# facebookresearch/AVID-CMA

Hardware: AMD Instinct MI355X
Metric: clips/sec (video+audio fwd+bwd+NCE+Adam) (higher is better)
Workload: dtype f32 (bf16x3 MFMA)

## Files before the change

### avid-cma_amd/csrc/conv.hip

```cpp
#include <math.h>
#include <stdlib.h>

#include <atomic>
#include <type_traits>

#include "common.h"

namespace avid {

typedef unsigned int uintx4 __attribute__((ext_vector_type(4)));

struct ConvArgs {
  const float* __restrict__ src;
  const float* __restrict__ wk;
  int w_row, w_nrec;
  const float* __restrict__ addend;
  const float* __restrict__ bias;
  float* __restrict__ dst;
  float* __restrict__ part;
  int B, Ts, Hs, Ws, Cs;
  int Td, Hd, Wd, Cd;
  int kt, kh, kw;
  int st, sh, sw;
  int pt, ph, pw;
// ... 704 lines not shown
#pragma unroll
        for (int j = 0; j < TN; ++j) {
          const pk_bf16x8 bh = bq[st & 1][j][0], bm = bq[st & 1][j][1], bl = bq[st & 1][j][2];
#pragma unroll
          for (int i = 0; i < TM; ++i) {
            acc[i][j] = __builtin_amdgcn_mfma_f32_32x32x16_bf16(ah[i], bl, acc[i][j], 0, 0, 0);
            acc[i][j] = __builtin_amdgcn_mfma_f32_32x32x16_bf16(al[i], bh, acc[i][j], 0, 0, 0);
            acc[i][j] = __builtin_amdgcn_mfma_f32_32x32x16_bf16(am[i], bm, acc[i][j], 0, 0, 0);
            acc[i][j] = __builtin_amdgcn_mfma_f32_32x32x16_bf16(ah[i], bm, acc[i][j], 0, 0, 0);
            acc[i][j] = __builtin_amdgcn_mfma_f32_32x32x16_bf16(am[i], bh, acc[i][j], 0, 0, 0);
            acc[i][j] = __builtin_amdgcn_mfma_f32_32x32x16_bf16(ah[i], bh, acc[i][j], 0, 0, 0);
          }
        }
      }
      return;
    }
    if (PK_SPLIT && TM * TN >= 4) {
      const float* As = Ab - h * 4 + h * 8;
      const float* Bs = Bb - h * 4 + h * 8;
#pragma unroll
      for (int st = 0; st < BK / 16; ++st) {
        if (decltype(ST)::value && st == 0) store_stage(nxt);
        if (decltype(LD)::value && st == 1) issue_loads();
        pk_bf16x8 ah[TM], am[TM], al[TM];
#pragma unroll
        for (int i = 0; i < TM; ++i) {
          const floatx4 v0 = *reinterpret_cast<const floatx4*>(As + i * 32 * LDK + st * 16);
          const floatx4 v1 = *reinterpret_cast<const floatx4*>(As + i * 32 * LDK + st * 16 + 4);
          pk_split8(v0, v1, ah[i], am[i], al[i]);
        }
#pragma unroll
        for (int j = 0; j < TN; ++j) {
          const floatx4 v0 = *reinterpret_cast<const floatx4*>(Bs + j * 32 * LDK + st * 16);
          const floatx4 v1 = *reinterpret_cast<const floatx4*>(Bs + j * 32 * LDK + st * 16 + 4);
          pk_bf16x8 bh, bm, bl;
          pk_split8(v0, v1, bh, bm, bl);
#pragma unroll
          for (int i = 0; i < TM; ++i) {
            acc[i][j] = __builtin_amdgcn_mfma_f32_32x32x16_bf16(ah[i], bl, acc[i][j], 0, 0, 0);
            acc[i][j] = __builtin_amdgcn_mfma_f32_32x32x16_bf16(al[i], bh, acc[i][j], 0, 0, 0);
            acc[i][j] = __builtin_amdgcn_mfma_f32_32x32x16_bf16(am[i], bm, acc[i][j], 0, 0, 0);
            acc[i][j] = __builtin_amdgcn_mfma_f32_32x32x16_bf16(ah[i], bm, acc[i][j], 0, 0, 0);
            acc[i][j] = __builtin_amdgcn_mfma_f32_32x32x16_bf16(am[i], bh, acc[i][j], 0, 0, 0);
            acc[i][j] = __builtin_amdgcn_mfma_f32_32x32x16_bf16(ah[i], bh, acc[i][j], 0, 0, 0);
          }
        }
      }
      return;
    }
    floatx4 af[2][TM], bf[2][TN];
#pragma unroll
    for (int i = 0; i < TM; ++i) af[0][i] = *reinterpret_cast<const floatx4*>(Ab + i * 32 * LDK);
#pragma unroll
    for (int j = 0; j < TN; ++j) bf[0][j] = *reinterpret_cast<const floatx4*>(Bb + j * 32 * LDK);
#pragma unroll
    for (int g = 0; g < BK / 8; ++g) {
      if (g + 1 < BK / 8) {
#pragma unroll
        for (int i = 0; i < TM; ++i)
          af[(g + 1) & 1][i] = *reinterpret_cast<const floatx4*>(Ab + i * 32 * LDK + (g + 1) * 8);
#pragma unroll
        for (int j = 0; j < TN; ++j)
          bf[(g + 1) & 1][j] = *reinterpret_cast<const floatx4*>(Bb + j * 32 * LDK + (g + 1) * 8);
      }
      __builtin_amdgcn_sched_barrier(0);
      if (decltype(ST)::value && g == 0) store_stage(nxt);
      if (decltype(LD)::value && g == 1) issue_loads();
#pragma unroll
      for (int s = 0; s < 4; ++s)
#pragma unroll
        for (int i = 0; i < TM; ++i)
#pragma unroll
          for (int j = 0; j < TN; ++j)
            acc[i][j] = __builtin_amdgcn_mfma_f32_32x32x2f32(af[g & 1][i][s], bf[g & 1][j][s], acc[i][j], 0, 0, 0);
      if (decltype(ST)::value && g == 0) {
#pragma unroll
        for (int q = 0; q < PA + PB; ++q) {
          __builtin_amdgcn_sched_group_barrier(0x008, 1, 0);
          __builtin_amdgcn_sched_group_barrier(0x200, 1, 0);
        }
      }
      if (decltype(LD)::value && g == 1) {
#pragma unroll
        for (int q = 0; q < PA + PB; ++q) {
          __builtin_amdgcn_sched_group_barrier(0x008, 1, 0);
          __builtin_amdgcn_sched_group_barrier(0x020, 1, 0);
        }
      }
      __builtin_amdgcn_sched_barrier(0);
    }
  };

  const int row_bytes = p.Cd * 4;
  for (int j = 0; j < nseg; ++j) {
    int tile, k0, k1, split;
    seg_info(j, tile, k0, k1, split);
    const int nkj = k1 - k0;
#pragma unroll
    for (int i = 0; i < TM; ++i)
#pragma unroll
      for (int jj = 0; jj < TN; ++jj)
#pragma unroll
        for (int r = 0; r < 16; ++r) acc[i][jj][r] = 0.f;

    int nst = left - 2 < nkj ? left - 2 : nkj;
    if (nst < 0) nst = 0;
    PK_STAMP(2 + 3 * j);
    for (int ks = 0; ks < nst; ++ks, u ^= 1) {
      ktile(std::true_type{}, std::true_type{});
      advance();
      __syncthreads();
    }
    left -= nst;
    if (nst < nkj) {
      if (left == 2) {
        ktile(std::true_type{}, std::false_type{});
        __syncthreads();
        u ^= 1;
        --left;
        ++nst;
      }
      if (nst < nkj) {
        ktile(std::false_type{}, std::false_type{});
        __syncthreads();
        u ^= 1;
        --left;
      }
    }

    PK_STAMP(3 + 3 * j);
    if (STRIDED) {
      int* drow = reinterpret_cast<int*>(smem + 2 * STAGE);
      int* arow = drow + BM;
      const bool sparse_add = p.add_s[0] * p.add_s[1] * p.add_s[2] > 1;
      const int c = cls_of(tile);
      const int lt = tile - kp->cls_begin[c];
      const int mt = lt / ntn, nt = lt - mt * ntn;
      const int n0 = nt * BN;
      const int cT = kp->cls_n[c][0], cH = kp->cls_n[c][1], cW = kp->cls_n[c][2];
      __syncthreads();
      if (tid < BM) {
        const unsigned m = mt * BM + tid;
        const bool ok = m < (unsigned)(p.B * cT * cH * cW);
        const unsigned mm = ok ? m : 0u;
        const unsigned q1 = magic_div(mm, kp->cls_mg[c][2], kp->cls_shf[c][2]);
        const int wd = mm - q1 * cW;
        const unsigned q2 = magic_div(q1, kp->cls_mg[c][1], kp->cls_shf[c][1]);
        const int hd = q1 - q2 * cH;
        const int b = magic_div(q2, kp->cls_mg[c][0], kp->cls_shf[c][0]);
        const int td = q2 - b * cT;
        const int dst = ((b * p.Td + kp->cls_p0[c][0] + td * p.st) * p.Hd + kp->cls_p0[c][1] + hd * p.sh) * p.Wd +
                        kp->cls_p0[c][2] + wd * p.sw;
        drow[tid] = ok ? dst * row_bytes : (int)OOB;
        if (sparse_add) {
          const int t = kp->cls_p0[c][0] + td * p.st, hh = kp->cls_p0[c][1] + hd * p.sh, w = kp->cls_p0[c][2] + wd * p.sw;
          const bool on = ok && (t & (p.add_s[0] - 1)) == 0 && (hh & (p.add_s[1] - 1)) == 0 && (w & (p.add_s[2] - 1)) == 0;
          const int ar = ((b * p.add_n[0] + (t >> (p.add_s[0] - 1))) * p.add_n[1] + (hh >> (p.add_s[1] - 1))) * p.add_n[2] +
                         (w >> (p.add_s[2] - 1));
          arow[tid] = on ? ar * row_bytes : (int)OOB;
        } else {
          arow[tid] = ok ? dst * row_bytes : (int)OOB;
        }
      }
      __syncthreads();
      const bool direct = split < 0;
      const __amdgpu_buffer_rsrc_t rsD = __builtin_amdgcn_make_buffer_rsrc(
          (void*)(direct ? p.dst : p.part + (long long)split * p.M * p.Cd), 0, (int)((long long)p.M * row_bytes), 0x00020000);
      const long long add_rows = sparse_add ? (long long)p.B * p.add_n[0] * p.add_n[1] * p.add_n[2] : (long long)p.M;
      const __amdgpu_buffer_rsrc_t rsE = __builtin_amdgcn_make_buffer_rsrc(
          (void*)(p.addend ? p.addend : p.dst), 0, (int)(add_rows * row_bytes), 0x00020000);
      const __amdgpu_buffer_rsrc_t rsXb = __builtin_amdgcn_make_buffer_rsrc(
          (void*)(p.bnb_x ? p.bnb_x : p.dst), 0, (int)((long long)p.M * row_bytes), 0x00020000);
      auto emit = [&](auto HAS_ADD, auto BNB) {
#pragma unroll
        for (int i = 0; i < TM; ++i) {
#pragma unroll
          for (int jj = 0; jj < TN; ++jj) {
            const int col = n0 + (wn * TN + jj) * 32 + l31;
            const int col4 = col * 4;
            unsigned voff[16];
            float ad[16], xb[16], bsc = 0.f, bsh = 0.f, bmu = 0.f, bis = 0.f;
#pragma unroll
            for (int r = 0; r < 16; ++r) {
              const int trow = (wm * TM + i) * 32 + (r & 3) + 8 * (r >> 2) + 4 * h;
              voff[r] = (unsigned)drow[trow] + col4;
              if (HAS_ADD)
                ad[r] = __builtin_bit_cast(float, __builtin_amdgcn_raw_buffer_load_b32(rsE, (unsigned)arow[trow] + col4, 0, 0));
              if (BNB) xb[r] = __builtin_bit_cast(float, __builtin_amdgcn_raw_buffer_load_b32(rsXb, voff[r], 0, 0));
            }
            if (BNB) { bsc = p.bnb_scale[col]; bsh = p.bnb_shift[col]; bmu = p.bnb_mean[col]; bis = p.bnb_invstd[col]; }
#pragma unroll
            for (int r = 0; r < 16; ++r) {
              float v = acc[i][jj][r];
              if (HAS_ADD) v += ad[r];
              if (BNB) {
                const float dm = (!p.bnb_relu || fmaf(xb[r], bsc, bsh) > 0.f) ? v : 0.f;
                cs[jj][r & 1] += dm;
                cq[jj][r & 1] = fmaf(dm, (xb[r] - bmu) * bis, cq[jj][r & 1]);
              }
              __builtin_amdgcn_raw_buffer_store_b32(__builtin_bit_cast(unsigned, v), rsD, voff[r], 0, 0);
            }
          }
        }
      };
      constexpr std::true_type Y{};
      constexpr std::false_type N{};
      if (!direct) emit(N, N);
      else if (EPI == 9) emit(Y, Y);
      else if (EPI == 8) emit(N, Y);
      else if (EPI == 1) emit(Y, N);
      else if (EPI == 0) emit(N, N);
      else if (p.bnb_x) { if (p.addend) emit(Y, Y); else emit(N, Y); }
      else if (p.addend) emit(Y, N);
      else emit(N, N);
      continue;
    }
    const int mt = tile / ntn, nt = tile - mt * ntn;
    const int m0 = mt * BM, n0 = nt * BN;
    int rows = p.M - m0;
    rows = rows > BM ? BM : rows;
    const bool direct = split < 0;
    const long long d_base = (long long)m0 * p.Cd;
    const long long s_base = ((long long)split * (p.M - p.part_row_begin) + (m0 - p.part_row_begin)) * p.Cd;
    const __amdgpu_buffer_rsrc_t rsD = __builtin_amdgcn_make_buffer_rsrc(
        (void*)(direct ? p.dst + d_base : p.part + s_base), 0, rows * row_bytes, 0x00020000);
    const __amdgpu_buffer_rsrc_t rsE = __builtin_amdgcn_make_buffer_rsrc(
        (void*)(p.addend ? p.addend + d_base : p.dst + d_base), 0, rows * row_bytes, 0x00020000);
    const __amdgpu_buffer_rsrc_t rsXb = __builtin_amdgcn_make_buffer_rsrc(
        (void*)(p.bnb_x ? p.bnb_x + d_base : p.dst + d_base), 0, rows * row_bytes, 0x00020000);
    auto emit = [&](auto DIRECT, auto HAS_ADD, auto RELU, auto OP, auto BNB, auto BIAS) {
#pragma unroll
      for (int i = 0; i < TM; ++i) {
#pragma unroll
        for (int jj = 0; jj < TN; ++jj) {
          const int col = n0 + (wn * TN + jj) * 32 + l31;
          const unsigned voff = (unsigned)(((wm * TM + i) * 32 + 4 * h) * p.Cd + col) * 4;
          float ad[16];
          if (HAS_ADD) {
#pragma unroll
            for (int r = 0; r < 16; ++r)
              ad[r] = __builtin_bit_cast(float, __builtin_amdgcn_raw_buffer_load_b32(
                                                    rsE, voff, ((r & 3) + 8 * (r >> 2)) * row_bytes, 0));
          }
          const float bv = (DIRECT && decltype(BIAS)::value != 0 && (decltype(BIAS)::value == 1 || p.bias)) ? p.bias[col] : 0.f;
          float xb[16], bsc = 0.f, bsh = 0.f, bmu = 0.f, bis = 0.f;
          if (BNB) {
#pragma unroll
            for (int r = 0; r < 16; ++r)
              xb[r] = __builtin_bit_cast(float, __builtin_amdgcn_raw_buffer_load_b32(
                                                    rsXb, voff, ((r & 3) + 8 * (r >> 2)) * row_bytes, 0));
            bsc = p.bnb_scale[col]; bsh = p.bnb_shift[col]; bmu = p.bnb_mean[col]; bis = p.bnb_invstd[col];
          }
#pragma unroll
          for (int r = 0; r < 16; ++r) {
            const int soff = ((r & 3) + 8 * (r >> 2)) * row_bytes;
            float v = acc[i][jj][r];
            if (DIRECT) {
              if (decltype(BIAS)::value != 0) v += bv;
              if (HAS_ADD) v = decltype(OP)::value == 0 ? v + ad[r] : (decltype(OP)::value == 1 ? fminf(v, ad[r]) : fmaxf(v, ad[r]));
              if (RELU) v = fmaxf(v, 0.f);
              if (MODE == 0) { cs[jj][r & 1] += v; cq[jj][r & 1] = fmaf(v, v, cq[jj][r & 1]); }
              if (BNB) {
                const float dm = (!p.bnb_relu || fmaf(xb[r], bsc, bsh) > 0.f) ? v : 0.f;
                cs[jj][r & 1] += dm;
                cq[jj][r & 1] = fmaf(dm, (xb[r] - bmu) * bis, cq[jj][r & 1]);
              }
            }
            __builtin_amdgcn_raw_buffer_store_b32(__builtin_bit_cast(unsigned, v), rsD, voff, soff, 0);
          }
        }
      }
    };
    constexpr std::true_type Y{};
    constexpr std::false_type N{};
    constexpr std::integral_constant<int, 0> ADD{};
    constexpr std::integral_constant<int, 0> B0{};
    constexpr std::integral_constant<int, 1> B1{};
    constexpr std::integral_constant<int, 2> BQ{};
    if (!direct) emit(N, N, N, ADD, N, B0);
    else if (EPI == 0) emit(Y, N, N, ADD, N, B0);
    else if (EPI == 1) emit(Y, Y, N, ADD, N, B0);
    else if (MODE == 0 && EPI == 2) emit(Y, N, N, ADD, N, B1);
    else if (MODE == 0 && EPI == 3) emit(Y, N, Y, ADD, N, B1);
    else if (MODE == 0 && EPI == 4) emit(Y, Y, N, std::integral_constant<int, 1>{}, N, B0);
    else if (MODE == 0 && EPI == 5) emit(Y, Y, N, std::integral_constant<int, 2>{}, N, B0);
    else if (MODE == 1 && EPI == 8) emit(Y, N, N, ADD, Y, B0);
    else if (MODE == 1 && EPI == 9) emit(Y, Y, N, ADD, Y, B0);
    else if (MODE == 1 && p.bnb_x) {
      if (p.addend) emit(Y, Y, N, ADD, Y, BQ); else emit(Y, N, N, ADD, Y, BQ);
    } else if (p.addend) {
      if (MODE == 0 && p.epi_op == 1) emit(Y, Y, N, std::integral_constant<int, 1>{}, N, BQ);
      else if (MODE == 0 && p.epi_op == 2) emit(Y, Y, N, std::integral_constant<int, 2>{}, N, BQ);
      else if (p.relu) emit(Y, Y, Y, ADD, N, BQ);
      else emit(Y, Y, N, ADD, N, BQ);
    } else {
      if (p.relu) emit(Y, N, Y, ADD, N, BQ); else emit(Y, N, N, ADD, N, BQ);
    }
    PK_STAMP(4 + 3 * j);
  }
  write_stats();
  PK_STAMP(31);
}

constexpr int WG_LD_C = 64 + 4;
constexpr int TC_P = 32;
constexpr int TC_T = 8;
constexpr int TC_ROWS = TC_P * TC_T;
constexpr int TC_B_BYTES = 6 * PK_BCH;
constexpr int TC_STAGE = TC_ROWS * LDK;
constexpr size_t TC_LDS = TC_B_BYTES + (2 * TC_STAGE + TC_P * LDK + 128) * sizeof(float);

template <int MODE, int EPI, bool AFF = false>
__global__ __launch_bounds__(512) __attribute__((amdgpu_waves_per_eu(2, 2))) void tconv64_kernel(const ConvArgs p) {
  constexpr bool OAFF = (EPI & 2) != 0;
  static_assert(!AFF || MODE == 0, "the input affine map belongs to the forward");
  static_assert(!OAFF || (MODE == 0 && (EPI & 8) == 0), "the output affine map belongs to the forward");
  extern __shared__ __attribute__((aligned(16))) float smem[];
  char* Bs = reinterpret_cast<char*>(smem);
  float* As = smem + TC_B_BYTES / 4;
  const int tid = threadIdx.x, lane = tid & 63;
  const int wave = __builtin_amdgcn_readfirstlane(tid >> 6);
  const int h = lane >> 5, l31 = lane & 31;
  const int lcol = (tid & 7) * 4;
  const int G = gridDim.x;
  const int slot = __builtin_amdgcn_readfirstlane((int)xcd_remap(blockIdx.x, G));
  PK_STAMP(0);
  const int HW = p.Hs * p.Ws;
  const int NP = p.B * HW;
  const int ntiles = (NP + TC_P - 1) / TC_P;
  const int nmine = slot < ntiles ? (ntiles - slot + G - 1) / G : 0;
  const int nitems = 2 * nmine;
  const int frame_bytes = HW * 256;

  float cs[2][2], cq[2][2];
#pragma unroll
  for (int j = 0; j < 2; ++j) cs[j][0] = cs[j][1] = cq[j][0] = cq[j][1] = 0.f;
  auto write_stats = [&]() {
    if (OAFF || !p.stats) return;
    float* red = As;
    __syncthreads();
#pragma unroll
    for (int j = 0; j < 2; ++j) {
      const float a0 = cs[j][0] + cs[j][1], b0 = cq[j][0] + cq[j][1];
      const float a = a0 + __shfl_xor(a0, 32, 64), b = b0 + __shfl_xor(b0, 32, 64);
      if (h == 0) {
        red[wave * 64 + j * 32 + l31] = a;
        red[512 + wave * 64 + j * 32 + l31] = b;
      }
    }
    __syncthreads();
    if (tid < 128) {
      const int c = tid & 63, which = tid >> 6;
      float a = 0.f;
#pragma unroll
      for (int w = 0; w < 8; ++w) a += red[which * 512 + w * 64 + c];
      p.stats[(long long)slot * 128 + which * 64 + c] = a;
      for (int r = slot + G; r < p.stats_rows; r += G) p.stats[(long long)r * 128 + which * 64 + c] = 0.f;
    }
  };
  if (nitems == 0) {
    write_stats();
    return;
  }

  const __amdgpu_buffer_rsrc_t rsA = __builtin_amdgcn_make_buffer_rsrc(
      (void*)p.src, 0, (int)((long long)p.M * 256), 0x00020000);
  const bool lead = wave < 4;
  const int trow = (tid & 255) >> 3;
  unsigned ld_voff = OOB;
  auto ld_tile = [&](int li) {
    const int tile = slot + (li >> 1) * G;
    const unsigned pg = (unsigned)(tile * TC_P + trow);
    const unsigned b = magic_div(pg, p.mgW, p.shW);
    const unsigned hw = pg - b * HW;
    ld_voff = pg < (unsigned)NP ? (unsigned)((b * TC_T * HW + hw) * 256 + lcol * 4) : OOB;
  };
  floatx4 va[8];
  auto issue_loads = [&](int li) {
    const int c128 = (li & 1) * 128;
#pragma unroll
    for (int i = 0; i < 8; ++i)
      va[i] = __builtin_bit_cast(floatx4, __builtin_amdgcn_raw_buffer_load_b128(
                                              rsA, ld_voff, __builtin_amdgcn_readfirstlane(c128 + i * frame_bytes), 0));
  };
  const float* aff = As + 2 * TC_STAGE + TC_P * LDK;
  auto store_stage = [&](float* st, int blk, bool first = false) {
    floatx4 asc = {0.f, 0.f, 0.f, 0.f}, ash = asc;
    if (AFF) {
      if (first) {
        asc = *reinterpret_cast<const floatx4*>(p.in_scale + blk * 32 + lcol);
        ash = *reinterpret_cast<const floatx4*>(p.in_shift + blk * 32 + lcol);
      } else {
        asc = *reinterpret_cast<const floatx4*>(aff + blk * 32 + lcol);
        ash = *reinterpret_cast<const floatx4*>(aff + 64 + blk * 32 + lcol);
      }
    }
#pragma unroll
    for (int i = 0; i < 8; ++i) {
      floatx4 v = va[i];
      if (AFF) {
        const bool ok = ld_voff != OOB;
#pragma unroll
        for (int j = 0; j < 4; ++j) {
          float o = fmaf(v[j], asc[j], ash[j]);
          if (p.in_relu) o = fmaxf(o, 0.f);
          v[j] = ok ? o : 0.f;
        }
      }
      *reinterpret_cast<floatx4*>(&st[(trow + 32 * i) * LDK + lcol]) = v;
    }
  };

  if (lead) {
    const __amdgpu_buffer_rsrc_t rsB = __builtin_amdgcn_make_buffer_rsrc(const_cast<void*>(p.wsp), 0, TC_B_BYTES, 0x00020000);
    pk_uintx4 wv[18];
#pragma unroll
    for (int i = 0; i < 18; ++i)
      wv[i] = __builtin_bit_cast(pk_uintx4, __builtin_amdgcn_raw_buffer_load_b128(rsB, (tid + 256 * i) * 16, 0, 0));
    for (int i = tid; i < TC_P * LDK; i += 256) As[2 * TC_STAGE + i] = 0.f;
    if (AFF && tid < 128) As[2 * TC_STAGE + TC_P * LDK + tid] = tid < 64 ? p.in_scale[tid] : p.in_shift[tid - 64];
#pragma unroll
    for (int i = 0; i < 18; ++i) *reinterpret_cast<pk_uintx4*>(Bs + (tid + 256 * i) * 16) = wv[i];
  } else {
    ld_tile(0);
    issue_loads(0);
    store_stage(As, 0, true);
    if (nitems > 1) issue_loads(1);
  }
  __syncthreads();

  floatx16 acc[2];
  const int row_bytes = 256;
  const __amdgpu_buffer_rsrc_t rsD = __builtin_amdgcn_make_buffer_rsrc((void*)p.dst, 0, (int)((long long)p.M * row_bytes), 0x00020000);
  const __amdgpu_buffer_rsrc_t rsE = __builtin_amdgcn_make_buffer_rsrc(
      (void*)(p.addend ? p.addend : p.dst), 0, (int)((long long)p.M * row_bytes), 0x00020000);
  const __amdgpu_buffer_rsrc_t rsXb = __builtin_amdgcn_make_buffer_rsrc(
      (void*)(p.bnb_x ? p.bnb_x : p.dst), 0, (int)((long long)p.M * row_bytes), 0x00020000);
  constexpr bool HAS_ADD = (EPI & 1) != 0, BNB = (EPI & 8) != 0;
  float bsc[2] = {0.f, 0.f}, bsh[2] = {0.f, 0.f}, bmu[2] = {0.f, 0.f}, bis[2] = {0.f, 0.f};
  if (BNB) {
#pragma unroll
    for (int j = 0; j < 2; ++j) {
      const int col = j * 32 + l31;
      bsc[j] = p.bnb_scale[col]; bsh[j] = p.bnb_shift[col]; bmu[j] = p.bnb_mean[col]; bis[j] = p.bnb_invstd[col];
    }
  }
  float osc[2] = {0.f, 0.f}, osh[2] = {0.f, 0.f};
  if (OAFF) {
#pragma unroll
    for (int j = 0; j < 2; ++j) {
      osc[j] = p.bnb_scale[j * 32 + l31];
      osh[j] = p.bnb_shift[j * 32 + l31];
    }
  }

  const float* Alane = As + l31 * LDK + h * 8;
  auto products = [&](int stage_off, auto CB) {
    constexpr int cb = decltype(CB)::value;
    int aoff[3];
#pragma unroll
    for (int d = 0; d < 3; ++d) {
      const int f = MODE == 0 ? wave + d - 1 : wave + 1 - d;
      aoff[d] = __builtin_amdgcn_readfirstlane((f < 0 || f >= TC_T) ? 2 * TC_STAGE : stage_off + f * TC_P * LDK);
    }
    const float* Af[3] = {Alane + aoff[0], Alane + aoff[1], Alane + aoff[2]};
    const char* Bc = Bs + cb * PK_BCH + lane * 16;
    floatx4 ar[3][2];
    pk_bf16x8 bf[3][6], sp[2][3];
    auto request = [&](int s_, int buf) {
      const int d = s_ >> 1, st = s_ & 1;
      ar[buf][0] = *reinterpret_cast<const floatx4*>(Af[d] + st * 16);
      ar[buf][1] = *reinterpret_cast<const floatx4*>(Af[d] + st * 16 + 4);
#pragma unroll
      for (int j = 0; j < 2; ++j)
#pragma unroll
        for (int t = 0; t < 3; ++t)
          bf[buf][j * 3 + t] = *reinterpret_cast<const pk_bf16x8*>(Bc + d * 2 * PK_BCH + ((j * 2 + st) * 3 + t) * 1024);
    };
    request(0, 0);
    request(1, 1);
    pk_split8<false>(ar[0][0], ar[0][1], sp[0][0], sp[0][1], sp[0][2]);
    __builtin_amdgcn_sched_barrier(0);
#pragma unroll
    for (int s_ = 0; s_ < 6; ++s_) {
      const int b = s_ % 3, q2 = s_ & 1;
      if (s_ + 2 < 6) request(s_ + 2, (s_ + 2) % 3);
      if (s_ + 1 < 6) pk_split8<false>(ar[(s_ + 1) % 3][0], ar[(s_ + 1) % 3][1], sp[q2 ^ 1][0], sp[q2 ^ 1][1], sp[q2 ^ 1][2]);
      const pk_bf16x8 ah = sp[q2][0], am = sp[q2][1], al = sp[q2][2];
      acc[0] = __builtin_amdgcn_mfma_f32_32x32x16_bf16(ah, bf[b][2], acc[0], 0, 0, 0);
      acc[1] = __builtin_amdgcn_mfma_f32_32x32x16_bf16(ah, bf[b][5], acc[1], 0, 0, 0);
      acc[0] = __builtin_amdgcn_mfma_f32_32x32x16_bf16(al, bf[b][0], acc[0], 0, 0, 0);
      acc[1] = __builtin_amdgcn_mfma_f32_32x32x16_bf16(al, bf[b][3], acc[1], 0, 0, 0);
      acc[0] = __builtin_amdgcn_mfma_f32_32x32x16_bf16(am, bf[b][1], acc[0], 0, 0, 0);
      acc[1] = __builtin_amdgcn_mfma_f32_32x32x16_bf16(am, bf[b][4], acc[1], 0, 0, 0);
      acc[0] = __builtin_amdgcn_mfma_f32_32x32x16_bf16(ah, bf[b][1], acc[0], 0, 0, 0);
      acc[1] = __builtin_amdgcn_mfma_f32_32x32x16_bf16(ah, bf[b][4], acc[1], 0, 0, 0);
      acc[0] = __builtin_amdgcn_mfma_f32_32x32x16_bf16(am, bf[b][0], acc[0], 0, 0, 0);
      acc[1] = __builtin_amdgcn_mfma_f32_32x32x16_bf16(am, bf[b][3], acc[1], 0, 0, 0);
      acc[0] = __builtin_amdgcn_mfma_f32_32x32x16_bf16(ah, bf[b][0], acc[0], 0, 0, 0);
      acc[1] = __builtin_amdgcn_mfma_f32_32x32x16_bf16(ah, bf[b][3], acc[1], 0, 0, 0);
      if (s_ + 2 < 6) __builtin_amdgcn_sched_group_barrier(0x100, 8, 0);
#pragma unroll
      for (int q = 0; q < 12; ++q) {
        __builtin_amdgcn_sched_group_barrier(0x008, 1, 0);
        if (s_ + 1 < 6) __builtin_amdgcn_sched_group_barrier(0x002, 3, 0);
      }
      __builtin_amdgcn_sched_barrier(0);
    }
  };

  auto emit = [&](int tile, const floatx16 (&res)[2], auto SPLIT) {
    const unsigned p0 = (unsigned)(tile * TC_P);
    const unsigned b0 = magic_div(p0, p.mgW, p.shW);
    const unsigned pb = (b0 + 1) * HW;
    const unsigned base = (p0 + (7 * b0 + wave) * HW) * 256u + l31 * 4 + h * 4 * 256;
    const unsigned step_b = 7u * HW * 256u;
    unsigned voff[16];
#pragma unroll
    for (int r = 0; r < 16; ++r) {
      voff[r] = base;
      if (decltype(SPLIT)::value) {
        const unsigned pg = p0 + (r & 3) + 8 * (r >> 2) + 4 * h;
        voff[r] = pg < (unsigned)NP ? base + (pg >= pb ? step_b : 0u) : OOB;
      }
    }
#pragma unroll
    for (int j = 0; j < 2; ++j) {
      float ad[16], xb[16];
      if (HAS_ADD) {
#pragma unroll
        for (int r = 0; r < 16; ++r)
          ad[r] = __builtin_bit_cast(float, __builtin_amdgcn_raw_buffer_load_b32(rsE, voff[r], ((r & 3) + 8 * (r >> 2)) * 256 + j * 128, 0));
      }
      if (BNB) {
#pragma unroll
        for (int r = 0; r < 16; ++r)
          xb[r] = __builtin_bit_cast(float, __builtin_amdgcn_raw_buffer_load_b32(rsXb, voff[r], ((r & 3) + 8 * (r >> 2)) * 256 + j * 128, 0));
      }
#pragma unroll
      for (int r = 0; r < 16; ++r) {
        float v = res[j][r];
        if (HAS_ADD) v += ad[r];
        if (OAFF) {
          v = fmaf(v, osc[j], osh[j]);
          if (p.bnb_relu) v = fmaxf(v, 0.f);
        } else if (MODE == 0) { cs[j][r & 1] += v; cq[j][r & 1] = fmaf(v, v, cq[j][r & 1]); }
        if (BNB) {
          const float dm = (!p.bnb_relu || fmaf(xb[r], bsc[j], bsh[j]) > 0.f) ? v : 0.f;
          cs[j][r & 1] += dm;
          cq[j][r & 1] = fmaf(dm, (xb[r] - bmu[j]) * bis[j], cq[j][r & 1]);
        }
        __builtin_amdgcn_raw_buffer_store_b32(__builtin_bit_cast(unsigned, v), rsD, voff[r], ((r & 3) + 8 * (r >> 2)) * 256 + j * 128, 0);
      }
    }
  };
  auto epilogue = [&](int tile, const floatx16 (&res)[2]) {
    const unsigned p0 = (unsigned)(tile * TC_P);
    const unsigned pb = (magic_div(p0, p.mgW, p.shW) + 1) * HW;
    if (p0 + TC_P <= pb && p0 + TC_P <= (unsigned)NP) emit(tile, res, std::false_type{});
    else emit(tile, res, std::true_type{});
  };
  auto stage_next = [&](int it, int cb) {
    if (it + 1 < nitems) store_stage(As + (cb ^ 1) * TC_STAGE, cb ^ 1);
    if (it + 2 < nitems) {
      if (cb == 0) ld_tile(it + 2);
      issue_loads(it + 2);
    }
  };
  floatx16 out[2];
  PK_STAMP(1);
  for (int t = 0; t < nmine; ++t) {
    PK_STAMP(2 + 7 * t);
    if (!lead) {
      stage_next(2 * t, 0);
      if (t > 0) epilogue(slot + (t - 1) * G, out);
    }
#pragma unroll
    for (int j = 0; j < 2; ++j)
#pragma unroll
      for (int r = 0; r < 16; ++r) acc[j][r] = 0.f;
    PK_STAMP(3 + 7 * t);
#ifdef AVID_PK_TRACE
    if (t == 3 && lane == 0) g_pk_trace[(512 + blockIdx.x) * 64 + wave] = wall_clock64();
#endif
    products(0, std::integral_constant<int, 0>{});
#ifdef AVID_PK_TRACE
    if (t == 3 && lane == 0) g_pk_trace[(512 + blockIdx.x) * 64 + 8 + wave] = wall_clock64();
#endif
    PK_STAMP(4 + 7 * t);
    __syncthreads();
    PK_STAMP(5 + 7 * t);
    if (!lead) stage_next(2 * t + 1, 1);
    products(TC_STAGE, std::integral_constant<int, 1>{});
    PK_STAMP(6 + 7 * t);
    if (lead) {
      epilogue(slot + t * G, acc);
    } else {
      out[0] = acc[0];
      out[1] = acc[1];
    }
    PK_STAMP(7 + 7 * t);
    __syncthreads();
    PK_STAMP(8 + 7 * t);
  }
  if (!lead) epilogue(slot + (nmine - 1) * G, out);
  PK_STAMP(31);
  write_stats();
}

constexpr int TWG_P = 16;
constexpr int TWG_PLANE = TC_T * TWG_P * WG_LD_C;
constexpr size_t TWG_LDS = sizeof(float) * 2 * 2 * TWG_PLANE;

struct TwgradArgs {
  const float* x; const float* dy; float* part;
  int B, HW;
  unsigned mg; int sh;
  const float* in_scale; const float* in_shift;
  int in_relu;
};

template <bool AFF>
__global__ __launch_bounds__(512) __attribute__((amdgpu_waves_per_eu(2, 2))) void twgrad64_kernel(const TwgradArgs p) {
  extern __shared__ __attribute__((aligned(16))) float smem[];
  const int tid = threadIdx.x, lane = tid & 63;
  const int wave = __builtin_amdgcn_readfirstlane(tid >> 6);
  const int h = lane >> 5, l31 = lane & 31;
  const int jn = wave & 1, jc = (wave >> 1) & 1, kh = wave >> 2;
  const int G = gridDim.x;
  const int slot = __builtin_amdgcn_readfirstlane((int)xcd_remap(blockIdx.x, G));
  const int HW = p.HW, NP = p.B * HW;
  const int ntiles = (NP + TWG_P - 1) / TWG_P;
  const int nmine = slot < ntiles ? (ntiles - slot + G - 1) / G : 0;
  const int frame_bytes = HW * 256;
  const long long total = (long long)NP * TC_T * 256;
  const __amdgpu_buffer_rsrc_t rsX = __builtin_amdgcn_make_buffer_rsrc((void*)p.x, 0, (int)total, 0x00020000);
  const __amdgpu_buffer_rsrc_t rsY = __builtin_amdgcn_make_buffer_rsrc((void*)p.dy, 0, (int)total, 0x00020000);
  const int trow = tid >> 4, lcol = (tid & 15) * 4;
  unsigned ld_voff = OOB;
  auto ld_tile = [&](int k) {
    const unsigned pg = (unsigned)((slot + k * G) * TWG_P + (trow & 15));
    const unsigned b = magic_div(pg, p.mg, p.sh);
    const unsigned hw = pg - b * HW;
    ld_voff = pg < (unsigned)NP ? (unsigned)(((b * TC_T + (trow >> 4)) * HW + hw) * 256 + lcol * 4) : OOB;
  };
  floatx4 vx[4], vy[4];
  auto issue_loads = [&]() {
#pragma unroll
    for (int i = 0; i < 4; ++i) {
      const int so = __builtin_amdgcn_readfirstlane(2 * i * frame_bytes);
      vy[i] = __builtin_bit_cast(floatx4, __builtin_amdgcn_raw_buffer_load_b128(rsY, ld_voff, so, 0));
      vx[i] = __builtin_bit_cast(floatx4, __builtin_amdgcn_raw_buffer_load_b128(rsX, ld_voff, so, 0));
    }
  };
  floatx4 asc = {0.f, 0.f, 0.f, 0.f}, ash = asc;
  if (AFF) {
    asc = *reinterpret_cast<const floatx4*>(p.in_scale + lcol);
    ash = *reinterpret_cast<const floatx4*>(p.in_shift + lcol);
  }
  auto store_stage = [&](float* st) {
#pragma unroll
    for (int i = 0; i < 4; ++i) {
      floatx4 v = vx[i];
      if (AFF) {
        const bool ok = ld_voff != OOB;
#pragma unroll
        for (int j = 0; j < 4; ++j) {
          float o = fmaf(v[j], asc[j], ash[j]);
          if (p.in_relu) o = fmaxf(o, 0.f);
          v[j] = ok ? o : 0.f;
        }
      }
      *reinterpret_cast<floatx4*>(&st[(trow + 32 * i) * WG_LD_C + lcol]) = vy[i];
      *reinterpret_cast<floatx4*>(&st[TWG_PLANE + (trow + 32 * i) * WG_LD_C + lcol]) = v;
    }
  };
  floatx16 acc[3];
#pragma unroll
  for (int d = 0; d < 3; ++d)
#pragma unroll
    for (int r = 0; r < 16; ++r) acc[d][r] = 0.f;
  if (nmine > 0) {
    ld_tile(0);
    issue_loads();
    store_stage(smem);
    if (nmine > 1) { ld_tile(1); issue_loads(); }
  }
  __syncthreads();
  auto frag = [&](const float* plane, int f, int col, pk_bf16x8& fh, pk_bf16x8& fm, pk_bf16x8& fl) {
    const float* q = plane + (f * TWG_P + h * 8) * WG_LD_C + col;
    float v[8];
#pragma unroll
    for (int i = 0; i < 8; ++i) v[i] = q[i * WG_LD_C];
    pk_split8<true>(floatx4{v[0], v[1], v[2], v[3]}, floatx4{v[4], v[5], v[6], v[7]}, fh, fm, fl);
  };
  const int ncol = jn * 32 + l31, ccol = jc * 32 + l31;
  const int t0 = kh * 4;
  for (int k = 0; k < nmine; ++k) {
    const float* cur = smem + (k & 1) * 2 * TWG_PLANE;
    float* nxt = smem + ((k + 1) & 1) * 2 * TWG_PLANE;
    if (k + 1 < nmine) store_stage(nxt);
    if (k + 2 < nmine) { ld_tile(k + 2); issue_loads(); }
    const float* Dp = cur;
    const float* Xp = cur + TWG_PLANE;
    pk_bf16x8 xw[3][3];
    if (t0 > 0) frag(Xp, t0 - 1, ccol, xw[0][0], xw[0][1], xw[0][2]);
    frag(Xp, t0, ccol, xw[1][0], xw[1][1], xw[1][2]);
#pragma unroll
    for (int tt = 0; tt < 4; ++tt) {
      const int t = t0 + tt;
      const int i0 = tt % 3, i1 = (tt + 1) % 3, i2 = (tt + 2) % 3;
      pk_bf16x8 ah, am, al;
      frag(Dp, t, ncol, ah, am, al);
      const bool has_next = t + 1 < TC_T;
      if (has_next) frag(Xp, t + 1, ccol, xw[i2][0], xw[i2][1], xw[i2][2]);
#pragma unroll
      for (int d = 0; d < 3; ++d) {
        const int sl = d == 0 ? i0 : (d == 1 ? i1 : i2);
        if ((d == 0 && t == 0) || (d == 2 && !has_next)) continue;
        const pk_bf16x8 bh = xw[sl][0], bm = xw[sl][1], bl = xw[sl][2];
        acc[d] = __builtin_amdgcn_mfma_f32_32x32x16_bf16(ah, bl, acc[d], 0, 0, 0);
        acc[d] = __builtin_amdgcn_mfma_f32_32x32x16_bf16(al, bh, acc[d], 0, 0, 0);
        acc[d] = __builtin_amdgcn_mfma_f32_32x32x16_bf16(am, bm, acc[d], 0, 0, 0);
        acc[d] = __builtin_amdgcn_mfma_f32_32x32x16_bf16(ah, bm, acc[d], 0, 0, 0);
        acc[d] = __builtin_amdgcn_mfma_f32_32x32x16_bf16(am, bh, acc[d], 0, 0, 0);
        acc[d] = __builtin_amdgcn_mfma_f32_32x32x16_bf16(ah, bh, acc[d], 0, 0, 0);
      }
    }
    __syncthreads();
  }
  float* xch = smem + (wave & 3) * (3 * 16 * 64);
  if (kh == 1) {
#pragma unroll
    for (int d = 0; d < 3; ++d)
#pragma unroll
      for (int r = 0; r < 16; ++r) xch[(d * 16 + r) * 64 + lane] = acc[d][r];
  }
  __syncthreads();
  if (kh == 0) {
    float* slab = p.part + (long long)slot * (64 * 3 * 64);
#pragma unroll
    for (int d = 0; d < 3; ++d)
#pragma unroll
      for (int r = 0; r < 16; ++r) {
        const int n = jn * 32 + (r & 3) + 8 * (r >> 2) + 4 * h;
        slab[(n * 3 + d) * 64 + ccol] = acc[d][r] + xch[(d * 16 + r) * 64 + lane];
      }
  }
}

__global__ __launch_bounds__(256) void splitk_reduce_kernel(const float* __restrict__ part, float* __restrict__ dst,
                                                            const float* __restrict__ addend,
                                                            const float* __restrict__ bias, long long n4, int G,
                                                            int nsplit, int relu) {
  const long long stride = (long long)gridDim.x * blockDim.x;
  for (long long i = (long long)blockIdx.x * blockDim.x + threadIdx.x; i < n4; i += stride) {
    floatx4 s = reinterpret_cast<const floatx4*>(part)[i];
    for (int k = 1; k < nsplit; ++k) s += reinterpret_cast<const floatx4*>(part)[(long long)k * n4 + i];
    if (bias) s += reinterpret_cast<const floatx4*>(bias)[i % G];
    if (addend) s += reinterpret_cast<const floatx4*>(addend)[i];
    if (relu) {
      s.x = fmaxf(s.x, 0.f); s.y = fmaxf(s.y, 0.f); s.z = fmaxf(s.z, 0.f); s.w = fmaxf(s.w, 0.f);
    }
    reinterpret_cast<floatx4*>(dst)[i] = s;
  }
}

__global__ __launch_bounds__(256) void splitk_reduce_stats_kernel(const float* __restrict__ part, float* __restrict__ dst,
                                                                  const float* __restrict__ addend, long long rows, int C,
                                                                  int nsplit, int rows_per_block,
                                                                  float* __restrict__ stats) {
  __shared__ floatx4 sh[2][256];
  const int G = C >> 2, tid = threadIdx.x;
  const int g = tid % G, r = tid / G, rpp = 256 / G;
  const long long n4 = rows * G;
  const long long row0 = (long long)blockIdx.x * rows_per_block;
  floatx4 s = {0, 0, 0, 0}, q = {0, 0, 0, 0};
  for (int k = r; k < rows_per_block; k += rpp) {
    const long long row = row0 + k;
    if (row >= rows) break;
    const long long i = row * G + g;
    floatx4 v = reinterpret_cast<const floatx4*>(part)[i];
    for (int j = 1; j < nsplit; ++j) v += reinterpret_cast<const floatx4*>(part)[(long long)j * n4 + i];
    if (addend) v += reinterpret_cast<const floatx4*>(addend)[i];
    reinterpret_cast<floatx4*>(dst)[i] = v;
    s += v;
    q += v * v;
  }
  sh[0][tid] = s;
  sh[1][tid] = q;
  __syncthreads();
  if (r == 0) {
    for (int k = 1; k < rpp; ++k) {
      s += sh[0][k * G + g];
      q += sh[1][k * G + g];
    }
    float* o = stats + (long long)blockIdx.x * 2 * C;
    *reinterpret_cast<floatx4*>(o + g * 4) = s;
    *reinterpret_cast<floatx4*>(o + C + g * 4) = q;
  }
}

__global__ __launch_bounds__(256) void splitk_reduce_bnb_kernel(const float* __restrict__ part, float* __restrict__ dst,
                                                                const float* __restrict__ addend, long long rows, int C,
                                                                int nsplit, int rows_per_block,
                                                                const float* __restrict__ x,
                                                                const float* __restrict__ scale,
                                                                const float* __restrict__ shift,
                                                                const float* __restrict__ mean,
                                                                const float* __restrict__ invstd, int relu,
                                                                float* __restrict__ stats) {
  __shared__ floatx4 sh[2][256];
  const int G = C >> 2, tid = threadIdx.x;
  const int g = tid % G, r = tid / G, rpp = 256 / G;
  const long long n4 = rows * G;
  const long long row0 = (long long)blockIdx.x * rows_per_block;
  const floatx4 sc = reinterpret_cast<const floatx4*>(scale)[g], sf = reinterpret_cast<const floatx4*>(shift)[g];
  const floatx4 mu = reinterpret_cast<const floatx4*>(mean)[g], is = reinterpret_cast<const floatx4*>(invstd)[g];
  floatx4 s = {0, 0, 0, 0}, q = {0, 0, 0, 0};
  for (int k = r; k < rows_per_block; k += rpp) {
    const long long row = row0 + k;
    if (row >= rows) break;
    const long long i = row * G + g;
    floatx4 v = reinterpret_cast<const floatx4*>(part)[i];
    for (int j = 1; j < nsplit; ++j) v += reinterpret_cast<const floatx4*>(part)[(long long)j * n4 + i];
    if (addend) v += reinterpret_cast<const floatx4*>(addend)[i];
    reinterpret_cast<floatx4*>(dst)[i] = v;
    const floatx4 xv = reinterpret_cast<const floatx4*>(x)[i];
    if (relu) {
#pragma unroll
      for (int j = 0; j < 4; ++j) v[j] = fmaf(xv[j], sc[j], sf[j]) > 0.f ? v[j] : 0.f;
    }
    s += v;
    q += v * ((xv - mu) * is);
  }
  sh[0][tid] = s;
  sh[1][tid] = q;
  __syncthreads();
  if (r == 0) {
    for (int k = 1; k < rpp; ++k) {
      s += sh[0][k * G + g];
      q += sh[1][k * G + g];
    }
    float* o = stats + (long long)blockIdx.x * 2 * C;
    *reinterpret_cast<floatx4*>(o + g * 4) = s;
    *reinterpret_cast<floatx4*>(o + C + g * 4) = q;
  }
}

struct ClsReduce {
  int Td, Hd, Wd;
  unsigned mgW, mgH, mgT;
  int shW, shH, shT;
  int pt, ph, pw;
  int s2t, s2h, s2w;
  int f_by_par[8];
  int add_s[3], add_n[3];
};

template <bool BNB>
__global__ __launch_bounds__(256) void splitk_reduce_cls_kernel(const float* __restrict__ part, float* __restrict__ dst,
                                                                const float* __restrict__ addend, long long rows, int C,
                                                                int rows_per_block, const ClsReduce cr,
                                                                const float* __restrict__ x,
                                                                const float* __restrict__ scale,
                                                                const float* __restrict__ shift,
                                                                const float* __restrict__ mean,
                                                                const float* __restrict__ invstd, int relu,
                                                                float* __restrict__ stats) {
  __shared__ floatx4 sh[2][256];
  const int G = C >> 2, tid = threadIdx.x;
  const int g = tid % G, r = tid / G, rpp = 256 / G;
  const long long n4 = rows * G;
  const long long row0 = (long long)blockIdx.x * rows_per_block;
  floatx4 sc = {0, 0, 0, 0}, sf = sc, mu = sc, is = sc;
  if (BNB) {
    sc = reinterpret_cast<const floatx4*>(scale)[g]; sf = reinterpret_cast<const floatx4*>(shift)[g];
    mu = reinterpret_cast<const floatx4*>(mean)[g]; is = reinterpret_cast<const floatx4*>(invstd)[g];
  }
  floatx4 s = {0, 0, 0, 0}, q = {0, 0, 0, 0};
  for (int k = r; k < rows_per_block; k += rpp) {
    const long long row = row0 + k;
    if (row >= rows) break;
    const unsigned m = (unsigned)row;
    const unsigned q1 = magic_div(m, cr.mgW, cr.shW);
    const int wd = m - q1 * cr.Wd;
    const unsigned q2 = magic_div(q1, cr.mgH, cr.shH);
    const int hd = q1 - q2 * cr.Hd;
    const unsigned b = magic_div(q2, cr.mgT, cr.shT);
    const int td = q2 - b * cr.Td;
    const int par = (cr.s2t ? ((td + cr.pt) & 1) << 2 : 0) | (cr.s2h ? ((hd + cr.ph) & 1) << 1 : 0) |
                    (cr.s2w ? ((wd + cr.pw) & 1) : 0);
    const int f = cr.f_by_par[par];
    if (f <= 1) continue;
    const long long i = row * G + g;
    floatx4 v = reinterpret_cast<const floatx4*>(part)[i];
    for (int j = 1; j < f; ++j) v += reinterpret_cast<const floatx4*>(part)[(long long)j * n4 + i];
    if (addend) {
      if (cr.add_s[0] * cr.add_s[1] * cr.add_s[2] > 1) {
        if (((td & (cr.add_s[0] - 1)) | (hd & (cr.add_s[1] - 1)) | (wd & (cr.add_s[2] - 1))) == 0) {
          const long long ar = (((long long)b * cr.add_n[0] + (td >> (cr.add_s[0] - 1))) * cr.add_n[1] + (hd >> (cr.add_s[1] - 1))) *
                                   cr.add_n[2] + (wd >> (cr.add_s[2] - 1));
          v += reinterpret_cast<const floatx4*>(addend)[ar * G + g];
        }
      } else {
        v += reinterpret_cast<const floatx4*>(addend)[i];
      }
    }
    reinterpret_cast<floatx4*>(dst)[i] = v;
    if (BNB) {
      const floatx4 xv = reinterpret_cast<const floatx4*>(x)[i];
      if (relu) {
#pragma unroll
        for (int j = 0; j < 4; ++j) v[j] = fmaf(xv[j], sc[j], sf[j]) > 0.f ? v[j] : 0.f;
      }
      s += v;
      q += v * ((xv - mu) * is);
    }
  }
  if (!BNB) return;
  sh[0][tid] = s;
  sh[1][tid] = q;
  __syncthreads();
  if (r == 0) {
    for (int k = 1; k < rpp; ++k) {
      s += sh[0][k * G + g];
      q += sh[1][k * G + g];
    }
    float* o = stats + (long long)blockIdx.x * 2 * C;
    *reinterpret_cast<floatx4*>(o + g * 4) = s;
    *reinterpret_cast<floatx4*>(o + C + g * 4) = q;
  }
}

template <int WM, int WN, int TM, int TN>
__global__ __launch_bounds__(256) void igemm_gather_kernel(const ConvArgs p) {
  constexpr int BM = WM * TM * 32, BN = WN * TN * 32;
  constexpr int PA = BM / 32, PB = BN / 32;
  extern __shared__ __attribute__((aligned(16))) float smem[];
  float* As = smem;
  float* Bs = smem + 2 * BM * LDK;
  int2* ktab = reinterpret_cast<int2*>(smem + 2 * (BM + BN) * LDK);

  const int tid = threadIdx.x, lane = tid & 63, wave = tid >> 6;
  const int wm = wave / WN, wn = wave % WN;
  const int lrow = tid >> 3, lcol = (tid & 7) * 4;
  const unsigned ntm = (p.M + BM - 1) / BM, ntn = p.Cd / BN;
  const unsigned tile = xcd_remap(blockIdx.x, ntm * ntn);
  const int m0 = (tile / ntn) * BM, n0 = (tile % ntn) * BN;
  const int ntaps = p.kt * p.kh * p.kw;
  const int K = ntaps * p.Cs;
  const int nk = (K + BK - 1) / BK;

  int a_t0[PA], a_h0[PA], a_w0[PA];
  long long a_base[PA];
#pragma unroll
  for (int i = 0; i < PA; ++i) {
    int b, td, hd, wd;
    bool ok;
    decode_row(m0 + lrow + 32 * i, p.M, p.Wd, p.Hd, p.Td, b, td, hd, wd, ok);
    a_t0[i] = td * p.st - p.pt;
    a_h0[i] = hd * p.sh - p.ph;
    a_w0[i] = wd * p.sw - p.pw;
    if (!ok) a_t0[i] = -(1 << 28);
    a_base[i] = (long long)b * p.ssB + (long long)a_t0[i] * p.ssT + (long long)a_h0[i] * p.ssH +
                (long long)a_w0[i] * p.ssW;
  }
  for (int k = tid; k < nk * BK; k += 256) {
    int2 e;
    if (k < K) {
      int tap = k / p.Cs, c = k - tap * p.Cs;
      int dw = tap % p.kw, r = tap / p.kw;
      int dh = r % p.kh, dt = r / p.kh;
      e.x = (int)(dt * p.ssT + dh * p.ssH + dw * p.ssW + c * p.ssC);
      e.y = dt | (dh << 8) | (dw << 16);
    } else {
      e.x = 0;
      e.y = -1;
    }
    ktab[k] = e;
  }
  __syncthreads();

  floatx4 va[PA], vb[PB];
  auto load_tile = [&](int ks) {
    const int kb = ks * BK + lcol;
    int2 e[4];
#pragma unroll
    for (int j = 0; j < 4; ++j) e[j] = ktab[kb + j];
#pragma unroll
    for (int i = 0; i < PA; ++i) {
      floatx4 v;
#pragma unroll
      for (int j = 0; j < 4; ++j) {
        const int dt = e[j].y & 0xff, dh = (e[j].y >> 8) & 0xff, dw = (e[j].y >> 16) & 0xff;
        const int ts = a_t0[i] + dt, hs = a_h0[i] + dh, ws = a_w0[i] + dw;
        const bool ok = (e[j].y >= 0) & ((unsigned)ts < (unsigned)p.Ts) & ((unsigned)hs < (unsigned)p.Hs) &
                        ((unsigned)ws < (unsigned)p.Ws);
        const float t = p.src[ok ? a_base[i] + e[j].x : 0];
        v[j] = ok ? t : 0.f;
      }
      va[i] = v;
    }
#pragma unroll
    for (int i = 0; i < PB; ++i) {
      const int n = n0 + lrow + 32 * i;
      floatx4 v;
#pragma unroll
      for (int j = 0; j < 4; ++j) {
        const float t = p.wk[(kb + j < K) ? (long long)n * K + kb + j : 0];
        v[j] = (kb + j < K) ? t : 0.f;
      }
      vb[i] = v;
    }
  };
  auto store_tile = [&](int buf) {
    float* Ab = As + buf * BM * LDK;
    float* Bb = Bs + buf * BN * LDK;
#pragma unroll
    for (int i = 0; i < PA; ++i) *reinterpret_cast<floatx4*>(&Ab[(lrow + 32 * i) * LDK + lcol]) = va[i];
#pragma unroll
    for (int i = 0; i < PB; ++i) *reinterpret_cast<floatx4*>(&Bb[(lrow + 32 * i) * LDK + lcol]) = vb[i];
  };

  floatx16 acc[TM][TN];
#pragma unroll
  for (int i = 0; i < TM; ++i)
#pragma unroll
    for (int j = 0; j < TN; ++j)
#pragma unroll
      for (int r = 0; r < 16; ++r) acc[i][j][r] = 0.f;
  const int h = lane >> 5, l31 = lane & 31;

  load_tile(0);
  store_tile(0);
  __syncthreads();
  for (int ks = 0; ks < nk; ++ks) {
    const int cur = ks & 1;
    if (ks + 1 < nk) load_tile(ks + 1);
    const float* Ab = As + cur * BM * LDK + (wm * TM * 32 + l31) * LDK + h * 4;
    const float* Bb = Bs + cur * BN * LDK + (wn * TN * 32 + l31) * LDK + h * 4;
#pragma unroll
    for (int g = 0; g < BK / 8; ++g) {
      floatx4 af[TM], bf[TN];
#pragma unroll
      for (int i = 0; i < TM; ++i) af[i] = *reinterpret_cast<const floatx4*>(Ab + i * 32 * LDK + g * 8);
#pragma unroll
      for (int j = 0; j < TN; ++j) bf[j] = *reinterpret_cast<const floatx4*>(Bb + j * 32 * LDK + g * 8);
#pragma unroll
      for (int s = 0; s < 4; ++s)
#pragma unroll
        for (int i = 0; i < TM; ++i)
// ... 2434 lines not shown
```

Measured before the change: 6642.

## Rewrite temporal wgrad kernel to stage bf16x3 split planes in LDS with transposed reads

Replaces the default temporal weight-gradient kernel with a version that splits x and dy into three bf16 planes once at load time and stores them in an LDS ring of three slots. Fragments are then fetched with ds_read_tr16 transposed reads, and the planes are laid out so that four pixel rows of a read hit each bank only once. Loading and splitting the next tile overlaps with the MFMAs on the current one. The old register-split version stays available behind a macro. The goal is to cut repeated per-fragment splitting and LDS bank conflicts, at the cost of more LDS and a more complex ring schedule with extra barriers.

```diff
diff --git a/avid-cma_amd/csrc/conv.hip b/avid-cma_amd/csrc/conv.hip
--- a/avid-cma_amd/csrc/conv.hip
+++ b/avid-cma_amd/csrc/conv.hip
@@ -1030,7 +1030,7 @@
   PK_STAMP(31);
 }
 
-constexpr int WG_LD_C = 64 + 4;
+[[maybe_unused]] constexpr int WG_LD_C = 64 + 4;
 constexpr int TC_P = 32;
 constexpr int TC_T = 8;
 constexpr int TC_ROWS = TC_P * TC_T;
@@ -1336,10 +1336,6 @@
   write_stats();
 }
 
-constexpr int TWG_P = 16;
-constexpr int TWG_PLANE = TC_T * TWG_P * WG_LD_C;
-constexpr size_t TWG_LDS = sizeof(float) * 2 * 2 * TWG_PLANE;
-
 struct TwgradArgs {
   const float* x; const float* dy; float* part;
   int B, HW;
@@ -1347,6 +1343,12 @@
   const float* in_scale; const float* in_shift;
   int in_relu;
 };
+
+#ifdef AVID_WGRAD_REGSPLIT
+constexpr int TWG_P = 16;
+constexpr int TWG_PLANE = TC_T * TWG_P * WG_LD_C;
+constexpr size_t TWG_LDS = sizeof(float) * 2 * 2 * TWG_PLANE;
+
 
 template <bool AFF>
 __global__ __launch_bounds__(512) __attribute__((amdgpu_waves_per_eu(2, 2))) void twgrad64_kernel(const TwgradArgs p) {
@@ -1476,6 +1478,198 @@
       }
   }
 }
+#else
+constexpr int TWG_P = 16;
+constexpr int TWG_HP = 8;
+constexpr int TWG_POS_B = TC_T * 64 * 2 + 64;
+constexpr int TWG_IMG_B = TWG_HP * TWG_POS_B;
+constexpr int TWG_SLOT_B = 2 * 3 * TWG_IMG_B;
+constexpr size_t TWG_LDS = 3 * TWG_SLOT_B;
+static_assert(TWG_LDS <= 160 * 1024 && TWG_LDS >= sizeof(float) * 4 * 3 * 16 * 64, "the ring and the final exchange fit the CU's LDS");
+static_assert(TWG_POS_B % 256 == 64 && TWG_IMG_B % 16 == 0, "four pixel rows of a transposed read cover the banks once");
+typedef __bf16 pk_bf16x4 __attribute__((ext_vector_type(4)));
+typedef unsigned pk_uintx2 __attribute__((ext_vector_type(2)));
+
+template <bool AFF>
+__global__ __launch_bounds__(512) __attribute__((amdgpu_waves_per_eu(2, 2))) void twgrad64_kernel(const TwgradArgs p) {
+  extern __shared__ __attribute__((aligned(16))) float smem[];
+  char* const lds = reinterpret_cast<char*>(smem);
+  const int tid = threadIdx.x, lane = tid & 63;
+  const int wave = __builtin_amdgcn_readfirstlane(tid >> 6);
+  const int h = lane >> 5, l31 = lane & 31;
+  const int jn = wave & 1, jc = (wave >> 1) & 1, kh = wave >> 2;
+  const int G = gridDim.x;
+  const int slot = __builtin_amdgcn_readfirstlane((int)xcd_remap(blockIdx.x, G));
+  const int HW = p.HW, NP = p.B * HW;
+  const int ntiles = (NP + TWG_P - 1) / TWG_P;
+  const int nmine = slot < ntiles ? (ntiles - slot + G - 1) / G : 0;
+  const int frame_bytes = HW * 256;
+  const long long total = (long long)NP * TC_T * 256;
+  const __amdgpu_buffer_rsrc_t rsX = __builtin_amdgcn_make_buffer_rsrc((void*)p.x, 0, (int)total, 0x00020000);
+  const __amdgpu_buffer_rsrc_t rsY = __builtin_amdgcn_make_buffer_rsrc((void*)p.dy, 0, (int)total, 0x00020000);
+  const int trow = tid >> 4, lcol = (tid & 15) * 4;
+  unsigned ld_voff[2] = {OOB, OOB};
+  auto ld_tile = [&](int k, auto S) {
+    constexpr int s = decltype(S)::value;
+    const unsigned pg = (unsigned)((slot + k * G) * TWG_P + s * TWG_HP + (trow & 7));
+    const unsigned b = magic_div(pg, p.mg, p.sh);
+    const unsigned hw = pg - b * HW;
+    ld_voff[s] = pg < (unsigned)NP ? (unsigned)(((b * TC_T + (trow >> 3)) * HW + hw) * 256 + lcol * 4) : OOB;
+  };
+  floatx4 vx[2][2], vy[2][2];
+  auto issue_loads = [&](auto S) {
+    constexpr int s = decltype(S)::value;
+#pragma unroll
+    for (int i = 0; i < 2; ++i) {
+      const int so = __builtin_amdgcn_readfirstlane(4 * i * frame_bytes);
+      vy[s][i] = __builtin_bit_cast(floatx4, __builtin_amdgcn_raw_buffer_load_b128(rsY, ld_voff[s], so, 0));
+      vx[s][i] = __builtin_bit_cast(floatx4, __builtin_amdgcn_raw_buffer_load_b128(rsX, ld_voff[s], so, 0));
+    }
+  };
+  floatx4 asc = {0.f, 0.f, 0.f, 0.f}, ash = asc;
+  if (AFF) {
+    asc = *reinterpret_cast<const floatx4*>(p.in_scale + lcol);
+    ash = *reinterpret_cast<const floatx4*>(p.in_shift + lcol);
+  }
+  struct HalfTerms { pk_uintx2 t[2][2][3]; };
+  auto split_half = [&](auto S, HalfTerms& o) {
+    constexpr int s = decltype(S)::value;
+#pragma unroll
+    for (int i = 0; i < 2; ++i) {
+      floatx4 v = vx[s][i];
+      if (AFF) {
+        const bool ok = ld_voff[s] != OOB;
+#pragma unroll
+        for (int j = 0; j < 4; ++j) {
+          float q = fmaf(v[j], asc[j], ash[j]);
+          if (p.in_relu) q = fmaxf(q, 0.f);
+          v[j] = ok ? q : 0.f;
+        }
+      }
+      const floatx4 y = vy[s][i];
+      unsigned a[3], b[3];
+      split2_bf16_dot(y[0], y[1], a[0], a[1], a[2]);
+      split2_bf16_dot(y[2], y[3], b[0], b[1], b[2]);
+#pragma unroll
+      for (int pl = 0; pl < 3; ++pl) o.t[0][i][pl] = pk_uintx2{a[pl], b[pl]};
+      split2_bf16_dot(v[0], v[1], a[0], a[1], a[2]);
+      split2_bf16_dot(v[2], v[3], b[0], b[1], b[2]);
+#pragma unroll
+      for (int pl = 0; pl < 3; ++pl) o.t[1][i][pl] = pk_uintx2{a[pl], b[pl]};
+    }
+  };
+  const int wr_off = (trow & 7) * TWG_POS_B + (trow >> 3) * 128 + lcol * 2;
+  auto write_half = [&](const HalfTerms& o, int ring) {
+    char* st = lds + ring * TWG_SLOT_B + wr_off;
+#pragma unroll
+    for (int op = 0; op < 2; ++op)
+#pragma unroll
+      for (int i = 0; i < 2; ++i)
+#pragma unroll
+        for (int pl = 0; pl < 3; ++pl)
+          *reinterpret_cast<pk_uintx2*>(st + (op * 3 + pl) * TWG_IMG_B + i * 4 * 128) = o.t[op][i][pl];
+  };
+  constexpr std::integral_constant<int, 0> HA{};
+  constexpr std::integral_constant<int, 1> HB{};
+  floatx16 acc[3];
+#pragma unroll
+  for (int d = 0; d < 3; ++d)
+#pragma unroll
+    for (int r = 0; r < 16; ++r) acc[d][r] = 0.f;
+  if (nmine > 0) {
+    HalfTerms ht;
+    ld_tile(0, HA); issue_loads(HA);
+    ld_tile(0, HB); issue_loads(HB);
+    split_half(HA, ht); write_half(ht, 0);
+    split_half(HB, ht); write_half(ht, 1);
+    ld_tile(1, HA); issue_loads(HA);
+    ld_tile(1, HB); issue_loads(HB);
+  }
+  __syncthreads();
+  typedef __attribute__((address_space(3))) pk_bf16x4 lds_bf16x4;
+  auto frag = [&](const char* img, int f, pk_bf16x8& fh, pk_bf16x8& fm, pk_bf16x8& fl) {
+    pk_bf16x8* const o[3] = {&fh, &fm, &fl};
+#pragma unroll
+    for (int pl = 0; pl < 3; ++pl) {
+      const char* q = img + pl * TWG_IMG_B + f * 128;
+      const pk_bf16x4 r0 = __builtin_amdgcn_ds_read_tr16_b64_v4bf16((lds_bf16x4*)(q));
+      const pk_bf16x4 r1 = __builtin_amdgcn_ds_read_tr16_b64_v4bf16((lds_bf16x4*)(q + 4 * TWG_POS_B));
+      *o[pl] = __builtin_shufflevector(r0, r1, 0, 1, 2, 3, 4, 5, 6, 7);
+    }
+  };
+  const int rd_off = ((lane & 15) >> 2) * TWG_POS_B + (lane & 16) * 2 + (lane & 3) * 8;
+  const int ccol = jc * 32 + l31;
+  const int t0 = kh * 4;
+  int ring = 0;
+  for (int k = 0; k < nmine; ++k) {
+    const int ringB = ring == 2 ? 0 : ring + 1, ringN = ringB == 2 ? 0 : ringB + 1;
+    const bool more = k + 1 < nmine;
+    HalfTerms hb;
+    if (more) {
+      HalfTerms ha;
+      split_half(HA, ha);
+      write_half(ha, ringN);
+    }
+    ld_tile(k + 2, HA); issue_loads(HA);
+    if (more) split_half(HB, hb);
+    ld_tile(k + 2, HB); issue_loads(HB);
+    const char* cur = lds + (h ? ringB : ring) * TWG_SLOT_B + rd_off;
+    const char* Dp = cur + jn * 64;
+    const char* Xp = cur + 3 * TWG_IMG_B + jc * 64;
+    pk_bf16x8 xw[4][3], a[2][3];
+    if (t0 > 0) frag(Xp, t0 - 1, xw[0][0], xw[0][1], xw[0][2]);
+    frag(Xp, t0, xw[1][0], xw[1][1], xw[1][2]);
+    frag(Dp, t0, a[0][0], a[0][1], a[0][2]);
+    frag(Xp, t0 + 1, xw[2][0], xw[2][1], xw[2][2]);
+#pragma unroll
+    for (int tt = 0; tt < 4; ++tt) {
+      const int t = t0 + tt;
+      const int i0 = tt & 3, i1 = (tt + 1) & 3, i2 = (tt + 2) & 3, i3 = (tt + 3) & 3;
+      const int ac = tt & 1, an = ac ^ 1;
+      const bool has_next = t + 1 < TC_T;
+      if (tt < 3) frag(Dp, t + 1, a[an][0], a[an][1], a[an][2]);
+      if (tt < 3 && t + 2 < TC_T) frag(Xp, t + 2, xw[i3][0], xw[i3][1], xw[i3][2]);
+      const pk_bf16x8 ah = a[ac][0], am = a[ac][1], al = a[ac][2];
+#pragma unroll
+      for (int d = 0; d < 3; ++d) {
+        const int sl = d == 0 ? i0 : (d == 1 ? i1 : i2);
+        if ((d == 0 && t == 0) || (d == 2 && !has_next)) continue;
+        const pk_bf16x8 bh = xw[sl][0], bm = xw[sl][1], bl = xw[sl][2];
+        acc[d] = __builtin_amdgcn_mfma_f32_32x32x16_bf16(ah, bl, acc[d], 0, 0, 0);
+        acc[d] = __builtin_amdgcn_mfma_f32_32x32x16_bf16(al, bh, acc[d], 0, 0, 0);
+        acc[d] = __builtin_amdgcn_mfma_f32_32x32x16_bf16(am, bm, acc[d], 0, 0, 0);
+        acc[d] = __builtin_amdgcn_mfma_f32_32x32x16_bf16(ah, bm, acc[d], 0, 0, 0);
+        acc[d] = __builtin_amdgcn_mfma_f32_32x32x16_bf16(am, bh, acc[d], 0, 0, 0);
+        acc[d] = __builtin_amdgcn_mfma_f32_32x32x16_bf16(ah, bh, acc[d], 0, 0, 0);
+      }
+    }
+    __syncthreads();
+    if (more) {
+      write_half(hb, ring);
+      __syncthreads();
+    }
+    ring = ringN;
+  }
+  float* xch = smem + (wave & 3) * (3 * 16 * 64);
+  if (kh == 1) {
+#pragma unroll
+    for (int d = 0; d < 3; ++d)
+#pragma unroll
+      for (int r = 0; r < 16; ++r) xch[(d * 16 + r) * 64 + lane] = acc[d][r];
+  }
+  __syncthreads();
+  if (kh == 0) {
+    float* slab = p.part + (long long)slot * (64 * 3 * 64);
+#pragma unroll
+    for (int d = 0; d < 3; ++d)
+#pragma unroll
+      for (int r = 0; r < 16; ++r) {
+        const int n = jn * 32 + (r & 3) + 8 * (r >> 2) + 4 * h;
+        slab[(n * 3 + d) * 64 + ccol] = acc[d][r] + xch[(d * 16 + r) * 64 + lane];
+      }
+  }
+}
+#endif
 
 __global__ __launch_bounds__(256) void splitk_reduce_kernel(const float* __restrict__ part, float* __restrict__ dst,
                                                             const float* __restrict__ addend,
```

Result: no change. 6643 (median of 2 runs) (+0.0%).
